# linyicheng1/trackingBench-SLAM

Hardware: AMD Instinct MI355X
Metric: frames/sec end-to-end (extract+match+local-BA) (higher is better)
Workload: dtype u8 (pyramid/FAST/ORB/Hamming) + f64 (pose-opt/BA); 1 GPU; 1280x720 stereo, 8-level pyramid x0.8, 2000 kpts/image (FAST 80/30), searchByBF L<->R, pose-opt, 10-KF/5000-pt local BA x10 iters; distinct_synthetic_pairs=64, distinct_ba_windows=32, ba_partitions=3, ba_schedule=joined at the end of every step, parallelism=frames sharded x1, RCCL gather of tracks

## Files before the change

### trackingbench_slam_amd/csrc/k_ba.hip

```cpp
#include <mutex>
#include <type_traits>
#include "tb_internal.h"
#include "tb_device.h"
#include "tb_se3.h"
#include "tb_math.h"

#define BA_T 256
#ifndef BA_KFCH
#define BA_KFCH 512
#endif
#ifndef BA_KFBLK
#define BA_KFBLK 4
#endif
#define BA_BIG_MAXF 64
#define BA_SMALL_MAXF 10
#define BA_SORT_LDS 8192
#ifndef BA_EMAX
#define BA_EMAX 64
#endif
#ifndef BA_UPD_BATCH
#define BA_UPD_BATCH 4
#endif
#ifndef BA_PCAP
#define BA_PCAP 21
#endif

struct BaState {
    double lambda, ni, currentChi, chi0, scale_p, rho;
    int iter, qmax, status, need_lin, cur, ok2, done_iters, err;
    int sing, pad0, hq_fresh, pad2;
};

struct BaDims {
    int W, nkf, nfixed, nfree, np, npt, obs_pitch, iters;
    int nblkP, kfChunks, G, nChunks;
    int Gbase, Gextra;
    int Vbase, Vextra;
    int big, npairs;
    unsigned long long oBigA;
    unsigned long long oPairStart, oPairCnt, oPairItems, maxItems;
    double fx, fy, cx, cy;
    unsigned long long wstride, oT, oP, oHll, oBl, oHq, oHpp, oBp, oXp, oPartKF, oPartP, oPartS;
    unsigned long long istride, oPtStart, oPtFree, oKfStart, oKfEdges, oFreeKP;
    unsigned long long oKfRec;
    unsigned long long oPtMask, oPermA, oPermB, oPtRank, oKPs, oGDesc;
    unsigned long long oGCost;
    unsigned long long oGCut;
    int renum;
    unsigned long long oPerm;
    int stream;
    int schurWaveLds;
    int wgReduce;
};

__host__ __device__ inline int ba_schur_waves(const BaDims& d, int w) {
    return d.wgReduce ? 4 * (d.Gbase + (w < d.Gextra ? 1 : 0)) : d.Vbase + (w < d.Vextra ? 1 : 0);
}
__device__ __forceinline__ void ba_schur_unit(int u, int base, int extra, int& w, int& i) {
    const int head = extra * (base + 1);
    if (u < head) { w = u / (base + 1); i = u - w * (base + 1); }
    else { const int r = u - head; w = extra + r / base; i = r - (w - extra) * base; }
}

typedef double ba_d4 __attribute__((ext_vector_type(4)));
typedef double ba_d2 __attribute__((ext_vector_type(2)));

__device__ __forceinline__ double ba_huber_rho0(double c, double delta) {
    const double dsqr = delta * delta;
    return (c <= dsqr) ? c : 2 * sqrt(c) * delta - dsqr;
}
struct BaLin { double ww, e0, e1, c2, invz; double pc[3]; double Jl[6]; };
__device__ __forceinline__ double ba_rcp(double x) {
    double r = __builtin_amdgcn_rcp(x);
    r = fma(fma(-x, r, 1.0), r, r);
    r = fma(fma(-x, r, 1.0), r, r);
    return r;
}
__device__ __forceinline__ void ba_residual(const double* Rt, const double* X, float u, float v, float inv_sigma2, double fx,
                                            double fy, double cx, double cy, double delta, BaLin& L) {
#pragma unroll
    for (int i = 0; i < 3; i++) L.pc[i] = fma(Rt[3 * i + 2], X[2], fma(Rt[3 * i + 1], X[1], fma(Rt[3 * i], X[0], Rt[9 + i])));
    L.invz = ba_rcp(L.pc[2]);
    L.e0 = (double)u - fma(L.pc[0] * L.invz, fx, cx);
    L.e1 = (double)v - fma(L.pc[1] * L.invz, fy, cy);
    const double wgt = (double)inv_sigma2;
    L.c2 = fma(L.e0, wgt * L.e0, L.e1 * (wgt * L.e1));
    const double r1 = (L.c2 <= delta * delta) ? 1.0 : delta / sqrt(L.c2);
    L.ww = r1 * wgt;
}
__device__ __forceinline__ void ba_linearize(const double* Rt, const double* X, float u, float v, float inv_sigma2, double fx,
                                             double fy, double cx, double cy, double delta, BaLin& L) {
    ba_residual(Rt, X, u, v, inv_sigma2, fx, fy, cx, cy, delta, L);
    const double ax = -(L.pc[0] * L.invz) * fx, ay = -(L.pc[1] * L.invz) * fy, m = -L.invz;
#pragma unroll
    for (int c = 0; c < 3; c++) {
        L.Jl[c] = m * fma(ax, Rt[6 + c], fx * Rt[c]);
        L.Jl[3 + c] = m * fma(ay, Rt[6 + c], fy * Rt[3 + c]);
    }
}
__device__ __forceinline__ void ba_pose_to_Rt(const double* T7, double* Rt) {
    PoSE3 s;
    s.qx = T7[0]; s.qy = T7[1]; s.qz = T7[2]; s.qw = T7[3]; s.tx = T7[4]; s.ty = T7[5]; s.tz = T7[6];
    po_to_R(s, Rt);
    Rt[9] = s.tx; Rt[10] = s.ty; Rt[11] = s.tz;
}
__device__ __forceinline__ void ba_jac_pose_iz(const double* pc, double invz, double fx, double fy, double* J) {
    const double xz = pc[0] * invz, yz = pc[1] * invz, xf = xz * fx, yf = yz * fy;
    J[0] = xf * yz; J[1] = -fma(xf, xz, fx); J[2] = yz * fx;
    J[3] = -invz * fx; J[4] = 0; J[5] = xf * invz;
    J[6] = fma(yf, yz, fy); J[7] = -(xz * yf); J[8] = -xz * fy;
    J[9] = 0; J[10] = -invz * fy; J[11] = yf * invz;
}

__device__ __forceinline__ bool ba_inv3(const double* H6, double lambda, double* I) {
    const double A0 = H6[0] + lambda, A1 = H6[1], A2 = H6[2], A4 = H6[3] + lambda, A5 = H6[4], A8 = H6[5] + lambda;
    const double A3 = A1, A6 = A2, A7 = A5;
    const double det = A0 * (A4 * A8 - A5 * A7) - A1 * (A3 * A8 - A5 * A6) + A2 * (A3 * A7 - A4 * A6);
    if (!(fabs(det) > 0)) return false;
    const double id = 1.0 / det;
    I[0] = (A4 * A8 - A5 * A7) * id; I[1] = (A2 * A7 - A1 * A8) * id; I[2] = (A1 * A5 - A2 * A4) * id;
    I[3] = (A5 * A6 - A3 * A8) * id; I[4] = (A0 * A8 - A2 * A6) * id; I[5] = (A2 * A3 - A0 * A5) * id;
    I[6] = (A3 * A7 - A4 * A6) * id; I[7] = (A1 * A6 - A0 * A7) * id; I[8] = (A0 * A4 - A1 * A3) * id;
    return true;
}
__device__ __forceinline__ PoSE3 ba_load_se3(const double* p) {
    PoSE3 s;
    s.qx = p[0]; s.qy = p[1]; s.qz = p[2]; s.qw = p[3]; s.tx = p[4]; s.ty = p[5]; s.tz = p[6];
    return s;
}
__device__ __forceinline__ void ba_store_se3(double* p, const PoSE3& s) {
    p[0] = s.qx; p[1] = s.qy; p[2] = s.qz; p[3] = s.qw; p[4] = s.tx; p[5] = s.ty; p[6] = s.tz;
}
__device__ __forceinline__ double ba_block_sum1(double v, double* red) {
    const int wave = threadIdx.x >> 6, lane = threadIdx.x & 63;
    v = po_wave_sum(v);
    __syncthreads();
    if (lane == 0) red[wave] = v;
    __syncthreads();
    return (red[0] + red[1]) + (red[2] + red[3]);
}
__device__ __forceinline__ double ba_block_max1(double v, double* red) {
    const int wave = threadIdx.x >> 6, lane = threadIdx.x & 63;
#pragma unroll
    for (int d = 32; d > 0; d >>= 1) v = fmax(v, __shfl_xor(v, d, 64));
    __syncthreads();
    if (lane == 0) red[wave] = v;
    __syncthreads();
    return fmax(fmax(red[0], red[1]), fmax(red[2], red[3]));
}

template <class Pred, class Pred2, class Visit>
__device__ __forceinline__ int ba_ordered_rank(int n, int* tmp, Pred pred, Pred2 pred2, int* total2, Visit visit) {
    const int wave = threadIdx.x >> 6, lane = threadIdx.x & 63;
    const int q = (((n + 3) >> 2) + 63) & ~63, lo = min(wave * q, n), hi = min(lo + q, n);
    int cnt = 0, cnt2 = 0;
    for (int e0 = lo; e0 < hi; e0 += 256) {
#pragma unroll
        for (int i = 0; i < 4; i++) {
            const int e = e0 + 64 * i + lane;
            cnt += (e < hi && pred(e)) ? 1 : 0;
            cnt2 += (e < hi && pred2(e)) ? 1 : 0;
        }
    }
    cnt = tb_wave_sum(cnt);
    cnt2 = tb_wave_sum(cnt2);
    if (lane == 0) { tmp[wave] = cnt; tmp[4 + wave] = cnt2; }
    __syncthreads();
    int base = 0;
    for (int v = 0; v < wave; v++) base += tmp[v];
    const int total = tmp[0] + tmp[1] + tmp[2] + tmp[3];
    *total2 = tmp[4] + tmp[5] + tmp[6] + tmp[7];
    const unsigned long long lt = (lane == 0) ? 0ull : (~0ull >> (64 - lane));
    for (int e0 = lo; e0 < hi; e0 += 256) {
        bool f[4];
#pragma unroll
        for (int i = 0; i < 4; i++) { const int e = e0 + 64 * i + lane; f[i] = e < hi && pred(e); }
#pragma unroll
        for (int i = 0; i < 4; i++) {
            const int e = e0 + 64 * i + lane;
            const unsigned long long m = __ballot(f[i]);
            if (e < hi) visit(e, base + __popcll(m & lt), f[i]);
            base += __popcll(m);
        }
    }
    __syncthreads();
    return total;
}

__global__ void __launch_bounds__(BA_T)
k_ba_setup(BaDims d, const float* __restrict__ poses, const float* __restrict__ pts, const tb_ba_obs* __restrict__ obsOrig,
           const tb_ba_obs* __restrict__ obsAll, const int32_t* __restrict__ obsCounts, double* __restrict__ dw, int* __restrict__ iw,
           BaState* __restrict__ states, int* __restrict__ errflag) {
    __shared__ int tmp[8];
    const int w = blockIdx.y, k = blockIdx.x, tid = threadIdx.x;
    const tb_ba_obs* obs = obsOrig + (size_t)w * d.obs_pitch;
    const int nobs = min(obsCounts[w], d.obs_pitch);
    double* D = dw + (size_t)w * d.wstride;
    int* I = iw + (size_t)w * d.istride;
    BaState* st = states + w;
    {
        const int nb = gridDim.x, per = (nobs + nb - 1) / nb;
        bool bad = false;
        for (int e = k * per + tid; e < min((k + 1) * per, nobs); e += BA_T) {
            const tb_ba_obs o = obs[e];
            if (o.kf < 0 || o.kf >= d.nkf || o.pt < 0 || o.pt >= d.npt || (e > 0 && o.pt < obs[e - 1].pt)) bad = true;
            for (int b0 = 1; b0 <= d.nkf && b0 <= e; b0 += 8) {
                int pk[8], pp[8];
#pragma unroll
                for (int i = 0; i < 8; i++) { const int ee = max(e - b0 - i, 0); pk[i] = obs[ee].kf; pp[i] = obs[ee].pt; }
#pragma unroll
                for (int i = 0; i < 8; i++)
                    if (b0 + i <= d.nkf && b0 + i <= e && pp[i] == o.pt && pk[i] == o.kf) bad = true;
                if (pp[7] != o.pt) break;
            }
        }
        if (bad) errflag[w] = 1;
    }
    obs = obsAll + (size_t)w * d.obs_pitch;
    if (d.renum && k != d.nkf) return;
    if (k < d.nkf) {
        int base = 0;
        const int mine = ba_ordered_rank(nobs, tmp, [&](int e) { return obs[e].kf == k; },
                                         [&](int e) { const int kf = obs[e].kf; return kf >= 0 && kf < k; }, &base,
                                         [&](int e, int rank, bool hit) {
                                             if (hit) {
                                                 I[d.oKfEdges + base + rank] = e;
                                                 const tb_ba_obs o = obs[e];
                                                 int4 r;
                                                 r.x = o.pt; r.y = __float_as_int(o.u); r.z = __float_as_int(o.v); r.w = __float_as_int(o.inv_sigma2);
                                                 *reinterpret_cast<int4*>(I + d.oKfRec + 4 * (size_t)(base + rank)) = r;
                                             }
                                         });
        if (tid == 0) {
            I[d.oKfStart + k] = base;
            if (k == d.nkf - 1) I[d.oKfStart + d.nkf] = base + mine;
        }
        return;
    }
    if (k == d.nkf + 1) {
        int unused = 0;
        const int nfreeE = ba_ordered_rank(nobs, tmp, [&](int e) { return obs[e].kf >= d.nfixed; }, [](int) { return false; }, &unused,
            [&](int e, int ce, bool hit) {
                const int prev = (e > 0) ? obs[e - 1].pt : -1, cur = obs[e].pt;
                for (int p = max(prev + 1, 0); p <= min(cur, d.npt); p++) I[d.oPtFree + p] = ce;
                if (hit) {
                    const tb_ba_obs o = obs[e];
                    int4 r;
                    r.x = (int)(((unsigned)cur << 6) | ((unsigned)(o.kf - d.nfixed) & 63u));
                    r.y = __float_as_int(o.u); r.z = __float_as_int(o.v); r.w = __float_as_int(o.inv_sigma2);
                    *reinterpret_cast<int4*>(I + d.oFreeKP + 4 * (size_t)ce) = r;
                }
            });
        for (int p = max((nobs > 0 ? obs[nobs - 1].pt : -1) + 1, 0) + tid; p <= d.npt; p += BA_T) I[d.oPtFree + p] = nfreeE;
        return;
    }
    if (tid == 0) {
        st->lambda = 0; st->ni = 2; st->currentChi = 0; st->chi0 = 0; st->scale_p = 0; st->rho = 0;
// ... 23 lines not shown
        D[d.oP + i] = v;
        D[d.oP + (size_t)d.npt * 3 + i] = v;
    }
}

__device__ __forceinline__ void ba_write_rec(double* q, const double* Hll, const double* bl, const double* X, double lambda,
                                             BaState* st) {
    const double a00 = Hll[0] + lambda, a10 = Hll[1], a20 = Hll[2], a11 = Hll[3] + lambda, a21 = Hll[4], a22 = Hll[5] + lambda;
    bool ok = a00 > 0;
    const double i00 = 1.0 / sqrt(ok ? a00 : 1.0), c10 = a10 * i00, c20 = a20 * i00;
    const double d1 = a11 - c10 * c10;
    ok = ok && d1 > 0;
    const double i11 = 1.0 / sqrt(ok ? d1 : 1.0), c21 = (a21 - c20 * c10) * i11;
    const double d2 = a22 - c20 * c20 - c21 * c21;
    ok = ok && d2 > 0 && isfinite(d2);
    const double i22 = 1.0 / sqrt(ok ? d2 : 1.0);
    if (!ok) st->sing = 1;
    const double u00 = i00, u11 = i11, u22 = i22, u01 = -c10 * i00 * i11, u12 = -c21 * i11 * i22,
                 u02 = -(c20 * i00 + c21 * u01) * i22;
    ba_d2* q2 = reinterpret_cast<ba_d2*>(q);
    q2[0] = ba_d2{ok ? u00 : 0.0, ok ? u01 : 0.0};
    q2[1] = ba_d2{ok ? u02 : 0.0, ok ? u11 : 0.0};
    q2[2] = ba_d2{ok ? u12 : 0.0, ok ? u22 : 0.0};
    q2[3] = ba_d2{bl[0], bl[1]};
    q2[4] = ba_d2{bl[2], X[0]};
    q2[5] = ba_d2{X[1], X[2]};
}
__device__ __forceinline__ void ba_load_rec(const double* __restrict__ q, double* __restrict__ r) {
    const ba_d2* q2 = reinterpret_cast<const ba_d2*>(q);
#pragma unroll
    for (int i = 0; i < 6; i++) { const ba_d2 v = q2[i]; r[2 * i] = v.x; r[2 * i + 1] = v.y; }
}

struct BaStreamPos { int base, deg; int4 first; };
template <class F>
__device__ __forceinline__ void ba_stream_walk(const int4* __restrict__ S, const BaStreamPos& sp, F f) {
    const int deg = sp.deg;
    int base = sp.base;
    unsigned long long m = __ballot(0 < deg);
    int4 rn = sp.first;
    for (int j = 0; m != 0; j++) {
        const int4 r = rn;
        const unsigned long long mn = __ballot(j + 1 < deg);
        const int idx = tbm::ba_stream_slot_self(mn, &base);
        if (j + 1 < deg) rn = S[idx];
        if (j < deg) f(r);
        m = mn;
    }
}
template <int N, class F>
__device__ __forceinline__ void ba_stream_walk_batched(const int4* __restrict__ S, const BaStreamPos& sp, F f) {
    const int deg = sp.deg;
    int base = sp.base - __popcll(__ballot(0 < deg));
    for (int j0 = 0; __ballot(j0 < deg) != 0; j0 += N) {
        int4 r[N];
#pragma unroll
        for (int i = 0; i < N; i++) {
            const unsigned long long m = __ballot(j0 + i < deg);
            const int idx = tbm::ba_stream_slot_self(m, &base);
            r[i] = make_int4(0, 0, 0, 0);
            if (j0 + i < deg) r[i] = S[idx];
        }
#pragma unroll
        for (int i = 0; i < N; i++)
            if (j0 + i < deg) f(r[i]);
    }
}
__device__ __forceinline__ BaStreamPos ba_stream_begin(const BaDims& d, const int* __restrict__ I, int p) {
    BaStreamPos sp;
    sp.base = I[d.oPtStart + min(p & ~63, d.npt)];
    sp.deg = (p < d.npt) ? I[d.oPtStart + p + 1] - I[d.oPtStart + p] : 0;
    sp.first = make_int4(0, 0, 0, 0);
    const int idx = tbm::ba_stream_slot_self(__ballot(0 < sp.deg), &sp.base);
    if (0 < sp.deg) sp.first = reinterpret_cast<const int4*>(I + d.oFreeKP)[idx];
    return sp;
}

__device__ __forceinline__ void ba_rec_utb(const double* q, double* t) {
    t[0] = q[0] * q[6];
    t[1] = q[1] * q[6] + q[3] * q[7];
    t[2] = q[2] * q[6] + q[4] * q[7] + q[5] * q[8];
}

template <bool STREAM>
__device__ __forceinline__ void ba_points_pass(const BaDims& d, const tb_ba_obs* __restrict__ obsAll, double* __restrict__ dw, const int* __restrict__ iw,
                                               BaState* __restrict__ states, const int* __restrict__ errflag, int bx, int w) {
    __shared__ double red[4];
    extern __shared__ __attribute__((aligned(16))) double sRt[];
    const int tid = threadIdx.x;
    double* D = dw + (size_t)w * d.wstride;
    const int* I = iw + (size_t)w * d.istride;
    const int p = bx * BA_T + tid;
    BaStreamPos sp;
    if (STREAM) sp = ba_stream_begin(d, I, p);
    if (errflag[w]) {
        if (bx == 0 && tid == 0) { states[w].status = 1; states[w].err = 1; }
        return;
    }
    const BaState st = states[w];
    if (st.status) return;
    const bool lam_known = st.iter > 0 || !st.need_lin;
    const tb_ba_obs* obs = obsAll + (size_t)w * d.obs_pitch;
    const double* T = D + d.oT + (size_t)st.cur * d.nkf * 7;
    const double* P = D + d.oP + (size_t)st.cur * d.npt * 3;
    for (int k = tid; k < d.nkf; k += BA_T) ba_pose_to_Rt(T + k * 7, sRt + k * 12);
    __syncthreads();
    const double delta = (double)sqrtf(5.991f);
    const bool in = p < d.npt;
    double chi = 0, maxd = 0;
    double Hll[6] = {0, 0, 0, 0, 0, 0}, bl[3] = {0, 0, 0}, X[3] = {0, 0, 0};
    if (in) { X[0] = P[3 * p]; X[1] = P[3 * p + 1]; X[2] = P[3 * p + 2]; }
    auto edge = [&](int kf, float ou, float ov, float ow) {
        BaLin L;
        ba_linearize(sRt + kf * 12, X, ou, ov, ow, d.fx, d.fy, d.cx, d.cy, delta, L);
        const double ww = L.ww, e0 = L.e0, e1 = L.e1;
        const double* Jl = L.Jl;
        chi += ba_huber_rho0(L.c2, delta);
        for (int a = 0; a < 3; a++) bl[a] = fma(-ww, fma(Jl[a], e0, Jl[3 + a] * e1), bl[a]);
        Hll[0] = fma(ww, fma(Jl[0], Jl[0], Jl[3] * Jl[3]), Hll[0]);
        Hll[1] = fma(ww, fma(Jl[0], Jl[1], Jl[3] * Jl[4]), Hll[1]);
        Hll[2] = fma(ww, fma(Jl[0], Jl[2], Jl[3] * Jl[5]), Hll[2]);
        Hll[3] = fma(ww, fma(Jl[1], Jl[1], Jl[4] * Jl[4]), Hll[3]);
        Hll[4] = fma(ww, fma(Jl[1], Jl[2], Jl[4] * Jl[5]), Hll[4]);
        Hll[5] = fma(ww, fma(Jl[2], Jl[2], Jl[5] * Jl[5]), Hll[5]);
    };
    if (STREAM) {
        ba_stream_walk(reinterpret_cast<const int4*>(I + d.oFreeKP), sp,
                       [&](const int4& r) { edge(r.x, __int_as_float(r.y), __int_as_float(r.z), __int_as_float(r.w)); });
    } else if (in) {
        const int eBeg = I[d.oPtStart + p], eEnd = I[d.oPtStart + p + 1];
        tb_ba_obs on = obs[min(eBeg, d.obs_pitch - 1)];
        for (int e = eBeg; e < eEnd; e++) {
            const tb_ba_obs o = on;
            on = obs[min(e + 1, d.obs_pitch - 1)];
            edge(o.kf, o.u, o.v, o.inv_sigma2);
        }
    }
    if (in) {
        if (!lam_known) {
            for (int a = 0; a < 6; a++) D[d.oHll + (size_t)p * 6 + a] = Hll[a];
            for (int a = 0; a < 3; a++) D[d.oBl + (size_t)p * 3 + a] = bl[a];
        } else
            ba_write_rec(D + d.oHq + (size_t)(d.renum ? p : I[d.oPtRank + p]) * 12, Hll, bl, X, st.lambda, states + w);
        maxd = fmax(fabs(Hll[0]), fmax(fabs(Hll[3]), fabs(Hll[5])));
    }
    const double s = ba_block_sum1(chi, red);
    const double m = ba_block_max1(maxd, red);
    if (tid == 0) {
        D[d.oPartP + (size_t)bx * 4] = s;
        D[d.oPartP + (size_t)bx * 4 + 1] = m;
    }
}

#define BA_KFG 14
#define BA_KFR_LDS (4 * (BA_KFG * 65 + 64) + 4 * 27)
__device__ __forceinline__ double ba_block_sum27(const double (&v)[27], double* sh) {
    const int tid = threadIdx.x, wave = tid >> 6, lane = tid & 63;
    double* T = sh + wave * (BA_KFG * 65 + 64);
    double* Qs = T + BA_KFG * 65;
    double* red = sh + 4 * (BA_KFG * 65 + 64);
#pragma unroll
    for (int g = 0; g < (27 + BA_KFG - 1) / BA_KFG; g++) {
        const int nv = min(BA_KFG, 27 - BA_KFG * g);
#pragma unroll
        for (int i = 0; i < BA_KFG; i++)
            if (i < nv) T[i * 65 + lane] = v[BA_KFG * g + i];
        __builtin_amdgcn_fence(__ATOMIC_SEQ_CST, "wavefront");
        const int q = lane / BA_KFG, i = lane - BA_KFG * q;
        if (lane < 4 * BA_KFG && i < nv) {
            const double* src = T + i * 65 + 16 * q;
            double s = src[0];
#pragma unroll
            for (int k = 1; k < 16; k++) s += src[k];
            Qs[lane] = s;
        }
        __builtin_amdgcn_fence(__ATOMIC_SEQ_CST, "wavefront");
        if (lane < nv) red[wave * 27 + BA_KFG * g + lane] = (Qs[lane] + Qs[BA_KFG + lane]) + (Qs[2 * BA_KFG + lane] + Qs[3 * BA_KFG + lane]);
        __builtin_amdgcn_fence(__ATOMIC_SEQ_CST, "wavefront");
    }
    __syncthreads();
    double r = 0;
    if (tid < 27) r = (red[tid] + red[27 + tid]) + (red[54 + tid] + red[81 + tid]);
    __syncthreads();
    return r;
}

__device__ __forceinline__ void ba_kf_pass(const BaDims& d, const tb_ba_obs* __restrict__ obsAll, double* __restrict__ dw, const int* __restrict__ iw,
                                           const BaState* __restrict__ states, const int* __restrict__ errflag, int bid) {
    __shared__ double red[BA_KFR_LDS];
    const int tid = threadIdx.x, nx = min(BA_KFBLK, d.kfChunks), per = nx * d.nfree;
    const int run = bid / (8 * per), rr_ = bid - run * (8 * per);
    const int w = run * 8 + (rr_ & 7), slot = rr_ >> 3;
    if (w >= d.W) return;
    if (errflag[w]) return;
    const int chunk0 = slot % nx, kfree = slot / nx, kf = d.nfixed + kfree;
    const BaState st = states[w];
    if (st.status || !st.need_lin) return;
    double* D = dw + (size_t)w * d.wstride;
    const int* I = iw + (size_t)w * d.istride;
    const int beg = I[d.oKfStart + kf], end = I[d.oKfStart + kf + 1];
    double Tk[12];
    ba_pose_to_Rt(D + d.oT + ((size_t)st.cur * d.nkf + kf) * 7, Tk);
    const double* P = D + d.oP + (size_t)st.cur * d.npt * 3;
    const double delta = (double)sqrtf(5.991f);
    for (int chunk = chunk0; chunk * BA_KFCH < end - beg; chunk += BA_KFBLK) {
        double acc[27];
#pragma unroll
        for (int i = 0; i < 27; i++) acc[i] = 0;
        int4 rr[BA_KFCH / BA_T];
        double XX[BA_KFCH / BA_T][3];
        const int4* KR = reinterpret_cast<const int4*>(I + d.oKfRec);
#pragma unroll
        for (int j = 0; j < BA_KFCH / BA_T; j++) {
            const int idx = beg + chunk * BA_KFCH + j * BA_T + tid;
            rr[j] = KR[min(idx, end - 1)];
            if (idx >= end) rr[j].x = -1;
        }
#pragma unroll
        for (int j = 0; j < BA_KFCH / BA_T; j++) {
            const int p = min(max(rr[j].x, 0), d.npt - 1);
            XX[j][0] = P[3 * p]; XX[j][1] = P[3 * p + 1]; XX[j][2] = P[3 * p + 2];
        }
#pragma unroll
        for (int j = 0; j < BA_KFCH / BA_T; j++) {
            if (rr[j].x < 0) continue;
            const float ou = __int_as_float(rr[j].y), ov = __int_as_float(rr[j].z), ow = __int_as_float(rr[j].w);
            const double* X = XX[j];
            double Jp[12];
            BaLin L;
            ba_residual(Tk, X, ou, ov, ow, d.fx, d.fy, d.cx, d.cy, delta, L);
            ba_jac_pose_iz(L.pc, L.invz, d.fx, d.fy, Jp);
            const double ww = L.ww, e0 = L.e0, e1 = L.e1;
#pragma unroll
            for (int a = 0; a < 6; a++) {
                const double wa = ww * Jp[a], wb = ww * Jp[6 + a];
                acc[21 + a] -= fma(wa, e0, wb * e1);
#pragma unroll
                for (int c = a; c < 6; c++) {
                    const int at = a * 6 - (a * (a - 1)) / 2 + (c - a);
                    acc[at] += fma(wa, Jp[c], wb * Jp[6 + c]);
                }
            }
        }
        const double tot = ba_block_sum27(acc, red);
        if (tid < 27) D[d.oPartKF + ((size_t)kfree * d.kfChunks + chunk) * 27 + tid] = tot;
    }
}

template <bool STREAM>
__global__ void __launch_bounds__(BA_T)
k_ba_points(BaDims d, const tb_ba_obs* __restrict__ obsAll, double* __restrict__ dw, const int* __restrict__ iw, BaState* __restrict__ states,
            const int* __restrict__ errflag) {
    ba_points_pass<STREAM>(d, obsAll, dw, iw, states, errflag, (int)blockIdx.x, (int)blockIdx.y);
}
__global__ void __launch_bounds__(BA_T)
k_ba_kf(BaDims d, const tb_ba_obs* __restrict__ obsAll, double* __restrict__ dw, const int* __restrict__ iw, const BaState* __restrict__ states,
        const int* __restrict__ errflag) {
    ba_kf_pass(d, obsAll, dw, iw, states, errflag, (int)blockIdx.x);
}
template <bool STREAM>
__global__ void __launch_bounds__(BA_T)
k_ba_lin(BaDims d, const tb_ba_obs* __restrict__ obsAll, double* __restrict__ dw, const int* __restrict__ iw, BaState* __restrict__ states,
         const int* __restrict__ errflag, int nKfBlocks) {
    if ((int)blockIdx.x < nKfBlocks) ba_kf_pass(d, obsAll, dw, iw, states, errflag, (int)blockIdx.x);
    else {
        const int b = (int)blockIdx.x - nKfBlocks;
        ba_points_pass<STREAM>(d, obsAll, dw, iw, states, errflag, b % d.nblkP, b / d.nblkP);
    }
}

__device__ __forceinline__ void ba_reduce_body(const BaDims& d, double* __restrict__ dw, const int* __restrict__ iw, BaState* __restrict__ states,
                                               int w, double* red) {
    const int tid = threadIdx.x;
    BaState* st = states + w;
    double* D = dw + (size_t)w * d.wstride;
    const int* I = iw + (size_t)w * d.istride;
    double maxd = 0;
    for (int i = tid; i < d.nfree * 27; i += BA_T) {
        const int kf = i / 27, c = i - kf * 27;
        const int nedges = I[d.oKfStart + d.nfixed + kf + 1] - I[d.oKfStart + d.nfixed + kf];
        const int nch = (nedges + BA_KFCH - 1) / BA_KFCH;
        double s = 0;
        for (int ch = 0; ch < nch; ch++) s += D[d.oPartKF + ((size_t)kf * d.kfChunks + ch) * 27 + c];
        if (c >= 21) D[d.oBp + kf * 6 + (c - 21)] = s;
        else {
            int a = 0, rem = c;
            while (rem >= 6 - a) { rem -= 6 - a; a++; }
            const int b = a + rem;
            D[d.oHpp + (size_t)kf * 36 + a * 6 + b] = s;
            D[d.oHpp + (size_t)kf * 36 + b * 6 + a] = s;
            if (a == b) maxd = fmax(maxd, fabs(s));
        }
    }
    const double mH = ba_block_max1(maxd, red);
    if (tid == 0) {
        double chi = 0, mL = 0;
        for (int b = 0; b < d.nblkP; b++) { chi += D[d.oPartP + (size_t)b * 4]; mL = fmax(mL, D[d.oPartP + (size_t)b * 4 + 1]); }
        st->currentChi = chi;
        if (st->iter == 0) { st->chi0 = chi; st->lambda = 1e-5 * fmax(mH, mL); st->ni = 2; }
        st->hq_fresh = st->iter > 0 ? 1 : 0;
        st->need_lin = 0;
    }
}

__global__ void __launch_bounds__(BA_T)
k_ba_reduce(BaDims d, double* __restrict__ dw, const int* __restrict__ iw, BaState* __restrict__ states) {
    __shared__ double red[4];
    const int w = blockIdx.x;
    if (states[w].status || !states[w].need_lin) return;
    ba_reduce_body(d, dw, iw, states, w, red);
}

__global__ void __launch_bounds__(BA_T)
k_ba_hinv(BaDims d, double* __restrict__ dw, const int* __restrict__ iw, BaState* __restrict__ states) {
    const int w = blockIdx.y, p = blockIdx.x * BA_T + threadIdx.x;
    const BaState st = states[w];
    if (st.status || st.hq_fresh || p >= d.npt) return;
    double* D = dw + (size_t)w * d.wstride;
    const int* I = iw + (size_t)w * d.istride;
    double ph[6], pb[3], X[3];
#pragma unroll
    for (int i = 0; i < 6; i++) ph[i] = D[d.oHll + (size_t)p * 6 + i];
#pragma unroll
    for (int i = 0; i < 3; i++) { pb[i] = D[d.oBl + (size_t)p * 3 + i]; X[i] = D[d.oP + ((size_t)st.cur * d.npt + p) * 3 + i]; }
    ba_write_rec(D + d.oHq + (size_t)(d.renum ? p : I[d.oPtRank + p]) * 12, ph, pb, X, st.lambda, states + w);
}

#define BA_MAXT 4
#define BA_REC 12
#define BA_RECS_LDS 256
#define BA_KMFMA 5
#define BA_ZERO_LDS 40
__device__ __forceinline__ void ba_wave_lds_fence() { __builtin_amdgcn_fence(__ATOMIC_SEQ_CST, "wavefront"); }

__host__ __device__ constexpr int ba_c_cap(int k) { return (BA_EMAX / k) < BA_PCAP ? (BA_EMAX / k) : BA_PCAP; }
__host__ __device__ constexpr int ba_c_nb(int k) { return (6 * k + 1 + 3) / 4; }
__host__ __device__ constexpr int ba_c_ld(int k) { return ((3 * ba_c_cap(k) + 3) / 4) * 4 + 2; }
__host__ __device__ constexpr int ba_c_tile(int k) { return 4 * ba_c_nb(k) * ba_c_ld(k); }
#define BA_CB 37
__host__ __device__ constexpr int ba_c_rhs(int k) { return BA_CB * (k * (k + 1) / 2); }
__host__ __device__ constexpr int ba_c_tri(int k) { return ba_c_rhs(k) + 6 * k; }
__host__ __device__ constexpr int ba_c_nacc(int k) {
    const int nb = ba_c_nb(k), nvf = nb / 4, rem = nb % 4;
    return 3 * nvf + 2 * nvf * (nvf - 1) + rem * (nvf + 1);
}
struct BaCTab { int cap[BA_SMALL_MAXF + 1], ld[BA_SMALL_MAXF + 1], nacc[BA_SMALL_MAXF + 1]; };
__host__ __device__ constexpr BaCTab ba_c_tab() {
    BaCTab t = {};
    for (int k = 1; k <= BA_SMALL_MAXF; k++) { t.cap[k] = ba_c_cap(k); t.ld[k] = ba_c_ld(k); t.nacc[k] = ba_c_nacc(k); }
    return t;
}
__device__ const BaCTab ba_ctab = ba_c_tab();
static int ba_c_wave_lds(int nfree) {
    int m = 0;
    for (int k = 1; k <= nfree; k++) m = std::max(m, std::max(ba_c_tile(k), k <= BA_KMFMA ? ba_c_tri(k) : 0));
    return ((m + 3) & ~3) + BA_RECS_LDS + BA_ZERO_LDS;
}

template <class IsZero>
__device__ __forceinline__ void ba_stable_split(int n, int* tmp, const int* src, int* dst, IsZero isZero) {
    const int wave = threadIdx.x >> 6, lane = threadIdx.x & 63;
    const int q = (((n + 3) >> 2) + 63) & ~63, lo = min(wave * q, n), hi = min(lo + q, n);
    int cnt = 0;
    for (int e = lo + lane; e < hi; e += 64) cnt += isZero(src[e]) ? 1 : 0;
    cnt = tb_wave_sum(cnt);
    if (lane == 0) tmp[wave] = cnt;
    __syncthreads();
    int z = 0;
    for (int v = 0; v < wave; v++) z += tmp[v];
    int o = (tmp[0] + tmp[1] + tmp[2] + tmp[3]) + (lo - z);
    const unsigned long long lt = (lane == 0) ? 0ull : (~0ull >> (64 - lane));
    for (int e0 = lo; e0 < hi; e0 += 64) {
        const int e = e0 + lane;
        const bool valid = e < hi;
        const int v = valid ? src[e] : 0;
        const bool f = valid && isZero(v);
        const unsigned long long m0 = __ballot(f), m1 = __ballot(valid && !f);
        if (valid) dst[f ? z + __popcll(m0 & lt) : o + __popcll(m1 & lt)] = v;
        z += __popcll(m0);
        o += __popcll(m1);
    }
    __threadfence_block();
    __syncthreads();
}

#define BA_RT 1024
#define BA_PREP_MAXKF 64
__global__ void __launch_bounds__(BA_RT)
k_ba_prepare(BaDims d, const tb_ba_obs* __restrict__ obsAll, const int32_t* __restrict__ obsCounts, int* __restrict__ iw,
             tb_ba_obs* __restrict__ obs2All) {
    extern __shared__ __attribute__((aligned(16))) unsigned prep_lds[];
    unsigned* word = prep_lds;
    int* first = reinterpret_cast<int*>(prep_lds + d.npt);
    int* start2 = first + d.npt;
    unsigned short* pbuf = reinterpret_cast<unsigned short*>(start2 + d.npt + 1);
    constexpr int NW = BA_RT / 64;
    __shared__ int tmp[NW + 2];
    __shared__ int bins[1 << BA_SMALL_MAXF];
    __shared__ int kfc[NW][BA_PREP_MAXKF];
    const int w = blockIdx.x, tid = threadIdx.x, wave = tid >> 6, lane = tid & 63;
    const unsigned long long lt = (lane == 0) ? 0ull : (~0ull >> (64 - lane));
    const tb_ba_obs* obs = obsAll + (size_t)w * d.obs_pitch;
    tb_ba_obs* obs2 = obs2All + (size_t)w * d.obs_pitch;
    const int nobs = min(max(obsCounts[w], 0), d.obs_pitch);
    int* I = iw + (size_t)w * d.istride;
    for (int p = tid; p < d.npt; p += BA_RT) { word[p] = 0; first[p] = 0; }
    for (int i = tid; i < (1 << BA_SMALL_MAXF); i += BA_RT) bins[i] = 0;
    __syncthreads();
    for (int e0 = tid; e0 < nobs; e0 += 4 * BA_RT) {
        tb_ba_obs o[4];
        int prev[4];
#pragma unroll
        for (int i = 0; i < 4; i++) {
            const int e = min(e0 + i * BA_RT, nobs - 1);
// ... 1486 lines not shown
static void ba_dims(BaDims& d, int num_cu, int peers, int W, const double K[4], int nkf, int nfixed, int npt, int obs_pitch, int iters) {
    memset(&d, 0, sizeof d);
    d.W = W; d.nkf = nkf; d.nfixed = nfixed; d.nfree = nkf - nfixed; d.np = 6 * d.nfree; d.npt = npt; d.obs_pitch = obs_pitch;
    d.iters = iters;
    d.nblkP = (npt + BA_T - 1) / BA_T;
    d.kfChunks = (obs_pitch + BA_KFCH - 1) / BA_KFCH;
    d.nChunks = 0;
    {
        const int slots = std::max(2 * std::max(num_cu, 1) / std::max(peers, 1), 1), cap = std::min(32, std::max((npt / 64 + 3) / 4, 1));
        d.Gbase = std::min(std::max(slots / std::max(W, 1), 1), cap);
        d.Gextra = (d.Gbase < cap && slots > d.Gbase * W) ? std::min(slots - d.Gbase * W, W) : 0;
        d.G = d.Gbase + (d.Gextra > 0 ? 1 : 0);
        d.wgReduce = d.Gbase > 4 ? 1 : 0;
        const int T = 4 * std::max(slots, W);
        d.Vbase = std::min(T / std::max(W, 1), 4 * cap);
        d.Vextra = d.Vbase < 4 * cap ? T % std::max(W, 1) : 0;
    }
    d.big = d.nfree > BA_SMALL_MAXF;
    d.renum = (!d.big && npt <= BA_SORT_LDS && nkf <= BA_PREP_MAXKF) ? 1 : 0;
    d.stream = d.renum;
    d.schurWaveLds = d.big ? 0 : ba_c_wave_lds(d.nfree);
    d.npairs = d.nfree * (d.nfree + 1) / 2;
    d.maxItems = (unsigned long long)obs_pitch * (d.nfree + 1) / 2 + 1;
    d.fx = K[0]; d.fy = K[1]; d.cx = K[2]; d.cy = K[3];
    unsigned long long o = 0;
    auto take = [&](unsigned long long n) { unsigned long long r = o; o += (n + 1) & ~1ull; return r; };
    d.oT = take(2ull * nkf * 7);
    d.oP = take(2ull * npt * 3);
    d.oHll = take(6ull * npt);
    d.oBl = take(3ull * npt);
    d.oHq = take(12ull * npt);
    d.oHpp = take(36ull * std::max(d.nfree, 1));
    d.oBp = take(std::max(64, d.np));
    d.oXp = take(std::max(64, d.np));
    d.oPartKF = take(27ull * std::max(d.nfree, 1) * d.kfChunks);
    d.oPartP = take(4ull * d.nblkP);
    const int maxWaves = d.wgReduce ? 4 * d.G : d.Vbase + (d.Vextra > 0 ? 1 : 0);
    d.oPartS = take(d.big ? 0 : 4096ull * (d.wgReduce ? d.G : maxWaves));
    d.oBigA = take(d.big ? (unsigned long long)(d.np + 1) * d.np + 32 : 0);
    d.wstride = o;
    unsigned long long io = 0;
    auto itake = [&](unsigned long long n) { unsigned long long r = io; io += (n + 3) & ~3ull; return r; };
    d.oPtStart = itake(npt + 1);
    d.oPtFree = itake(npt + 1);
    d.oKfStart = itake(nkf + 1);
    d.oKfEdges = itake(obs_pitch);
    d.oFreeKP = itake(4ull * obs_pitch);
    d.oKfRec = itake(4ull * obs_pitch);
    d.oPtRank = itake(npt);
    d.oPerm = itake(d.renum ? npt : 0);
    d.oPtMask = itake(d.big ? 0 : npt);
    d.oPermA = itake(d.big ? 0 : npt);
    d.oPermB = itake(d.big ? 0 : npt);
    d.oKPs = itake(d.big ? 0 : 4ull * obs_pitch);
    d.oGDesc = itake(d.big ? 0 : 4ull * npt + 4);
    d.oGCost = itake(d.big ? 0 : (unsigned long long)npt + 1);
    d.oGCut = itake(d.big ? 0 : (unsigned long long)maxWaves + 1);
    d.oPairStart = itake(d.big ? d.npairs + 1 : 0);
    d.oPairCnt = itake(d.big ? d.npairs : 0);
    d.oPairItems = itake(d.big ? 2 * d.maxItems : 0);
    d.istride = io;
}

#define BA_RING 1000

struct BaPlan {
    BaDims d;
    float *poses, *pts;
    const tb_ba_obs* obs_in;
    const int32_t* counts;
    void* work;
    double* dw;
    int* iw;
    BaState* states;
    int *running, *errflag;
    tb_ba_obs* obs2;
    size_t work_bytes;
    const tb_ba_obs* obs;
    decltype(&k_ba_schur_c<1>) schur;
    decltype(&k_ba_solve<16>) solve;
    decltype(&k_ba_lin<true>) lin;
    decltype(&k_ba_points<true>) points;
    decltype(&k_ba_update<true>) update;
    size_t prepare_lds, pass_lds, schur_lds, big_lds, update_lds;
};

static BaPlan ba_plan(const tb_ctx* ctx, int W, const double K[4], int nkf, int nfixed, int npt, int obs_pitch, int iters, float* d_poses,
                      float* d_pts, const tb_ba_obs* d_obs, const int32_t* d_counts, void* d_work) {
    BaPlan p;
    BaDims& d = p.d;
    ba_dims(d, ctx->num_cu, ctx->peers, W, K, nkf, nfixed, npt, obs_pitch, iters);
    if (ctx->dbg_ba_plain_obs) d.stream = 0;
    p.poses = d_poses; p.pts = d_pts; p.obs_in = d_obs; p.counts = d_counts; p.work = d_work;
    uintptr_t at = (uintptr_t)d_work;
    size_t total = 0;
    auto take = [&](size_t bytes, size_t align) {
        at = (at + align - 1) / align * align;
        const uintptr_t r = at;
        at += bytes;
        total += bytes + (align > 1 ? align : 0);
        return r;
    };
    p.dw = (double*)take((size_t)W * d.wstride * sizeof(double), 1);
    p.iw = (int*)take((size_t)W * d.istride * sizeof(int), 1);
    p.states = (BaState*)take((size_t)W * sizeof(BaState), 1);
    p.running = (int*)take(BA_RING * sizeof(int), 1);
    p.errflag = (int*)take((size_t)W * sizeof(int), 1);
    p.obs2 = d.renum ? (tb_ba_obs*)take((size_t)W * obs_pitch * sizeof(tb_ba_obs), 64) : nullptr;
    p.work_bytes = total + 96;
    p.obs = d.renum ? p.obs2 : d_obs;
    const int R = (d.np + 15) >> 4;
    p.schur = R == 1 ? k_ba_schur_c<1> : R == 2 ? k_ba_schur_c<2> : R == 3 ? k_ba_schur_c<3> : k_ba_schur_c<4>;
    p.solve = d.np <= 16 ? k_ba_solve<16> : d.np <= 32 ? k_ba_solve<32> : d.np <= 48 ? k_ba_solve<48> : k_ba_solve<64>;
    p.lin = d.stream ? k_ba_lin<true> : k_ba_lin<false>;
    p.points = d.stream ? k_ba_points<true> : k_ba_points<false>;
    p.update = d.stream ? k_ba_update<true> : k_ba_update<false>;
    p.prepare_lds = (size_t)npt * 16 + 16;
    p.pass_lds = (size_t)d.nkf * 12 * sizeof(double);
    p.schur_lds = std::max<size_t>(4 * (size_t)d.schurWaveLds, d.wgReduce ? 64 * 64 : 0) * sizeof(double);
    p.big_lds = (size_t)(d.np + 1) * BA_PLD * sizeof(double);
    p.update_lds = ((size_t)d.nkf * 24 + d.np) * sizeof(double);
    return p;
}

size_t tbk_local_ba_work_bytes(const tb_ctx* ctx, int W, int nkf, int nfixed, int npt, int obs_pitch) {
    const double K[4] = {1, 1, 0, 0};
    return ba_plan(ctx, W, K, nkf, nfixed, npt, obs_pitch, 1, nullptr, nullptr, nullptr, nullptr, nullptr).work_bytes;
}

static int ba_enqueue_head(tb_ctx* ctx, const BaPlan& p) {
    const BaDims& d = p.d;
    const int W = d.W;
    TB_TRY(tb_launch(ctx, nullptr, k_ba_zero, dim3((BA_RING + W + 255) / 256), dim3(256), 0, p.running, BA_RING + W));
    if (d.renum) TB_TRY(tb_launch(ctx, "k_ba_prepare", k_ba_prepare, dim3(W), dim3(BA_RT), p.prepare_lds, d, p.obs_in, p.counts, p.iw, p.obs2));
    TB_TRY(tb_launch(ctx, "k_ba_setup", k_ba_setup, dim3(d.nkf + 2, W), dim3(BA_T), 0, d, p.poses, p.pts, p.obs_in, p.obs, p.counts, p.dw, p.iw,
                     p.states, p.errflag));
    if (d.renum) {
    } else if (!d.big) {
        TB_TRY(tb_launch(ctx, "k_ba_groups", k_ba_groups, dim3(W), dim3(BA_T), 0, d, p.iw, p.errflag));
    } else {
        tb_prof_begin(ctx, "k_ba_pairs");
        TB_TRY(tb_launch(ctx, nullptr, k_ba_pairs<false>, dim3(d.nfree, W), dim3(64), 0, d, p.obs, p.iw, p.errflag));
        TB_TRY(tb_launch(ctx, nullptr, k_ba_pair_scan, dim3(W), dim3(BA_T), 0, d, p.iw, p.errflag));
        TB_TRY(tb_launch(ctx, nullptr, k_ba_pairs<true>, dim3(d.nfree, W), dim3(64), 0, d, p.obs, p.iw, p.errflag));
        tb_prof_end(ctx);
    }
    return TB_OK;
}

static int ba_enqueue_round(tb_ctx* ctx, const BaPlan& p, int round) {
    const BaDims& d = p.d;
    const int W = d.W;
    const int nKfBlocks = ((W + 7) / 8) * 8 * std::min(BA_KFBLK, d.kfChunks) * d.nfree;
    if (W <= 32) {
        TB_TRY(tb_launch(ctx, "k_ba_lin", p.lin, dim3(nKfBlocks + d.nblkP * W), dim3(BA_T), p.pass_lds, d, p.obs, p.dw, p.iw, p.states, p.errflag,
                         nKfBlocks));
    } else {
        TB_TRY(tb_launch(ctx, "k_ba_points", p.points, dim3(d.nblkP, W), dim3(BA_T), p.pass_lds, d, p.obs, p.dw, p.iw, p.states, p.errflag));
        TB_TRY(tb_launch(ctx, "k_ba_kf", k_ba_kf, dim3(nKfBlocks), dim3(BA_T), 0, d, p.obs, p.dw, p.iw, p.states, p.errflag));
    }
    const bool reduce_in_solve = !d.big && round > 0;
    if (!reduce_in_solve) TB_TRY(tb_launch(ctx, "k_ba_reduce", k_ba_reduce, dim3(W), dim3(BA_T), 0, d, p.dw, p.iw, p.states));
    if (round == 0)
        TB_TRY(tb_launch(ctx, "k_ba_hinv", k_ba_hinv, dim3(d.nblkP, W), dim3(BA_T), 0, d, p.dw, p.iw, p.states));
    if (d.big) {
        TB_TRY(tb_launch(ctx, "k_ba_schur_pairs", k_ba_schur_pairs, dim3((d.npairs + 3) / 4, W), dim3(BA_T), 0, d, p.dw, p.iw, p.states));
        TB_TRY(tb_launch(ctx, "k_ba_solve_big", k_ba_solve_big, dim3(W), dim3(BA_ST), p.big_lds, d, p.dw, p.states));
    } else {
        TB_TRY(tb_launch(ctx, "k_ba_schur", p.schur, dim3(d.wgReduce ? d.Gbase * W + d.Gextra : (d.Vbase * W + d.Vextra + 3) / 4), dim3(BA_T),
                         p.schur_lds, d, p.dw, p.iw, p.states));
        TB_TRY(tb_launch(ctx, "k_ba_solve", p.solve, dim3(W), dim3(BA_SOLVE_T), 0, d, p.dw, p.iw, p.states, reduce_in_solve ? 1 : 0));
    }
    TB_TRY(tb_launch(ctx, "k_ba_update", p.update, dim3(d.nblkP, W), dim3(BA_T), p.update_lds, d, p.obs, p.dw, p.iw, p.states));
    return tb_launch(ctx, "k_ba_decide", k_ba_decide, dim3(W), dim3(64), 0, d, p.dw, p.states, p.running + round % BA_RING);
}

static int ba_graph(tb_ctx* ctx, const BaPlan& p, int nfirst, hipGraphExec_t* exec) {
    struct Key { BaDims d; const void *poses, *pts, *obs, *counts, *work; hipStream_t s; } key;
    memset(&key, 0, sizeof key);
    key.d = p.d; key.poses = p.poses; key.pts = p.pts; key.obs = p.obs_in; key.counts = p.counts; key.work = p.work; key.s = ctx->stream;
    const std::string kb((const char*)&key, sizeof key);
    for (auto& g : ctx->ba_graphs)
        if (g.first == kb) { *exec = g.second; return TB_OK; }
    static std::mutex capture_lock;
    std::lock_guard<std::mutex> guard(capture_lock);
    hipGraph_t graph = nullptr;
    TB_HIP(ctx, hipStreamBeginCapture(ctx->stream, hipStreamCaptureModeThreadLocal));
    int rc = ba_enqueue_head(ctx, p);
    for (int r = 0; r < nfirst && rc == TB_OK; r++) rc = ba_enqueue_round(ctx, p, r);
    const hipError_t e = hipStreamEndCapture(ctx->stream, &graph);
    if (rc != TB_OK) { if (graph) hipGraphDestroy(graph); return rc; }
    TB_HIP(ctx, e);
    const hipError_t e2 = hipGraphInstantiate(exec, graph, nullptr, nullptr, 0);
    hipGraphDestroy(graph);
    TB_HIP(ctx, e2);
    if (ctx->ba_graphs.size() >= 8) {
        hipGraphExecDestroy(ctx->ba_graphs.front().second);
        ctx->ba_graphs.erase(ctx->ba_graphs.begin());
    }
    ctx->ba_graphs.emplace_back(kb, *exec);
    return TB_OK;
}

int tbk_local_ba_batch(tb_ctx* ctx, int W, const double K[4], int nkf, int nfixed, float* d_poses, int npt, float* d_pts,
                       const tb_ba_obs* d_obs, const int32_t* d_counts, int obs_pitch, int iters, double* d_stats, void* d_work,
                       size_t work_bytes) {
    if (W <= 0) return TB_OK;
    const int nfree = nkf - nfixed;
    if (nfree < 1 || nfree > BA_BIG_MAXF)
        return tb_fail(ctx, TB_EUNSUPPORTED, "local BA: %d free keyframes (this build supports 1..64)", nfree);
    if (nkf > TB_MAX_LEVELS * 8) return tb_fail(ctx, TB_EUNSUPPORTED, "local BA: too many keyframes");
    if (npt > (1 << 25)) return tb_fail(ctx, TB_EUNSUPPORTED, "local BA: more than 2^25 points per window");
    if (nfree > BA_SMALL_MAXF && (unsigned long long)obs_pitch * (nfree + 1) >= (1ull << 31))
        return tb_fail(ctx, TB_EUNSUPPORTED, "local BA: large window with more than 2^31 / (free keyframes + 1) observations");
    if (iters > 99) return tb_fail(ctx, TB_EUNSUPPORTED, "local BA: more than 99 LM iterations (one still-running counter per trial, 1000 of them)");
    const BaPlan p = ba_plan(ctx, W, K, nkf, nfixed, npt, obs_pitch, iters, d_poses, d_pts, d_obs, d_counts, d_work);
    const BaDims& d = p.d;
    if (p.work_bytes > work_bytes) return tb_fail(ctx, TB_ENOMEM, "local BA workspace too small");
    hipStream_t s = ctx->stream;
    if (!d.big) TB_TRY(tb_lds_limit(ctx, (const void*)p.schur, p.schur_lds));
    if (d.renum) TB_TRY(tb_lds_limit(ctx, (const void*)k_ba_prepare, p.prepare_lds));
    if (d.big) TB_TRY(tb_lds_limit(ctx, (const void*)k_ba_solve_big, p.big_lds));
    const int max_rounds = std::min(iters * 10 + 1, BA_RING);
    int batch = iters;
    const int nfirst = std::min(batch, max_rounds);
    const bool use_graph = W <= 32 && !ctx->prof && nfirst > 0;
    int rounds = 0;
    if (use_graph) {
        hipGraphExec_t exec = nullptr;
        TB_TRY(ba_graph(ctx, p, nfirst, &exec));
        TB_HIP(ctx, hipGraphLaunch(exec, s));
        rounds = nfirst;
    } else {
        TB_TRY(ba_enqueue_head(ctx, p));
    }
    int host_running = nfirst > 0 ? 1 : 0;
    bool replayed = use_graph;
    while (host_running > 0 && (rounds < max_rounds || replayed)) {
        if (!replayed)
            for (int r = 0; r < batch && rounds < max_rounds; r++, rounds++) TB_TRY(ba_enqueue_round(ctx, p, rounds));
        replayed = false;
        TB_HIP(ctx, hipMemcpyAsync(&host_running, p.running + (rounds - 1) % BA_RING, sizeof(int), hipMemcpyDeviceToHost, s));
        TB_HIP(ctx, hipStreamSynchronize(s));
        batch = 4;
    }
    return tb_launch(ctx, "k_ba_finish", k_ba_finish, dim3(W), dim3(BA_T), 0, d, p.dw, p.iw, p.states, d_poses, d_pts, d_stats);
}
```

Measured before the change: 34190 frames/s.

## Restructure BA keyframe pass into contiguous chunk ranges with prefetch pipelining

The keyframe Hessian pass now gives each block a contiguous range of chunks (one block per keyframe by default) instead of striding chunks across four blocks. Within that range it streams edge records through a two-deep software prefetch of records and point gathers, accumulating into a single register accumulator. The keyframe pose is computed once per block, shared through LDS and made wave-uniform with readfirstlane. The reduction group size is shrunk, launch bounds now request occupancy, and unused partial slots are zeroed. This is meant to cut redundant reductions and latency stalls, at the cost of fewer blocks and less parallelism per keyframe.

```diff
diff --git a/trackingbench_slam_amd/csrc/k_ba.hip b/trackingbench_slam_amd/csrc/k_ba.hip
--- a/trackingbench_slam_amd/csrc/k_ba.hip
+++ b/trackingbench_slam_amd/csrc/k_ba.hip
@@ -10,7 +10,19 @@
 #define BA_KFCH 512
 #endif
 #ifndef BA_KFBLK
-#define BA_KFBLK 4
+#define BA_KFBLK 1
+#endif
+#ifndef BA_KFE
+#define BA_KFE 2
+#endif
+#ifndef BA_LIN_FUSE_ALL
+#define BA_LIN_FUSE_ALL 0
+#endif
+#ifndef BA_KF_AHEAD
+#define BA_KF_AHEAD 1
+#endif
+#ifndef BA_KF_POSE_ONCE
+#define BA_KF_POSE_ONCE 1
 #endif
 #define BA_BIG_MAXF 64
 #define BA_SMALL_MAXF 10
@@ -103,6 +115,10 @@
     s.qx = T7[0]; s.qy = T7[1]; s.qz = T7[2]; s.qw = T7[3]; s.tx = T7[4]; s.ty = T7[5]; s.tz = T7[6];
     po_to_R(s, Rt);
     Rt[9] = s.tx; Rt[10] = s.ty; Rt[11] = s.tz;
+}
+__device__ __forceinline__ double ba_uniform(double v) {
+    const int lo = __builtin_amdgcn_readfirstlane(__double2loint(v)), hi = __builtin_amdgcn_readfirstlane(__double2hiint(v));
+    return __hiloint2double(hi, lo);
 }
 __device__ __forceinline__ void ba_jac_pose_iz(const double* pc, double invz, double fx, double fy, double* J) {
     const double xz = pc[0] * invz, yz = pc[1] * invz, xf = xz * fx, yf = yz * fy;
@@ -432,13 +448,16 @@
     }
 }
 
-#define BA_KFG 14
-#define BA_KFR_LDS (4 * (BA_KFG * 65 + 64) + 4 * 27)
+#ifndef BA_KFG
+#define BA_KFG 4
+#endif
+#define BA_KFW_LDS (BA_KFG * 65 + 4 * BA_KFG)
+#define BA_KFR_LDS (4 * BA_KFW_LDS + 4 * 27)
 __device__ __forceinline__ double ba_block_sum27(const double (&v)[27], double* sh) {
     const int tid = threadIdx.x, wave = tid >> 6, lane = tid & 63;
-    double* T = sh + wave * (BA_KFG * 65 + 64);
+    double* T = sh + wave * BA_KFW_LDS;
     double* Qs = T + BA_KFG * 65;
-    double* red = sh + 4 * (BA_KFG * 65 + 64);
+    double* red = sh + 4 * BA_KFW_LDS;
 #pragma unroll
     for (int g = 0; g < (27 + BA_KFG - 1) / BA_KFG; g++) {
         const int nv = min(BA_KFG, 27 - BA_KFG * g);
@@ -467,44 +486,67 @@
 
 __device__ __forceinline__ void ba_kf_pass(const BaDims& d, const tb_ba_obs* __restrict__ obsAll, double* __restrict__ dw, const int* __restrict__ iw,
                                            const BaState* __restrict__ states, const int* __restrict__ errflag, int bid) {
-    __shared__ double red[BA_KFR_LDS];
+    __shared__ double red[BA_KFR_LDS + 12];
     const int tid = threadIdx.x, nx = min(BA_KFBLK, d.kfChunks), per = nx * d.nfree;
     const int run = bid / (8 * per), rr_ = bid - run * (8 * per);
     const int w = run * 8 + (rr_ & 7), slot = rr_ >> 3;
     if (w >= d.W) return;
     if (errflag[w]) return;
-    const int chunk0 = slot % nx, kfree = slot / nx, kf = d.nfixed + kfree;
+    const int share = slot % nx, kfree = slot / nx, kf = d.nfixed + kfree;
     const BaState st = states[w];
     if (st.status || !st.need_lin) return;
     double* D = dw + (size_t)w * d.wstride;
     const int* I = iw + (size_t)w * d.istride;
     const int beg = I[d.oKfStart + kf], end = I[d.oKfStart + kf + 1];
+    const int nch = (end - beg + BA_KFCH - 1) / BA_KFCH, cps = (nch + nx - 1) / nx;
+    const int c0 = share * cps, c1 = min(c0 + cps, nch);
+    if (c0 >= c1) return;
+    const int eb = beg + c0 * BA_KFCH, ee = min(beg + c1 * BA_KFCH, end);
     double Tk[12];
+#if BA_KF_POSE_ONCE
+    double* sRt = red + BA_KFR_LDS;
+    if (tid < 64) {
+        ba_pose_to_Rt(D + d.oT + ((size_t)st.cur * d.nkf + kf) * 7, Tk);
+        if (tid == 0) {
+#pragma unroll
+            for (int i = 0; i < 12; i++) sRt[i] = Tk[i];
+        }
+    }
+    __syncthreads();
+#pragma unroll
+    for (int i = 0; i < 12; i++) Tk[i] = ba_uniform(sRt[i]);
+#else
     ba_pose_to_Rt(D + d.oT + ((size_t)st.cur * d.nkf + kf) * 7, Tk);
+#pragma unroll
+    for (int i = 0; i < 12; i++) Tk[i] = ba_uniform(Tk[i]);
+#endif
     const double* P = D + d.oP + (size_t)st.cur * d.npt * 3;
     const double delta = (double)sqrtf(5.991f);
-    for (int chunk = chunk0; chunk * BA_KFCH < end - beg; chunk += BA_KFBLK) {
-        double acc[27];
-#pragma unroll
-        for (int i = 0; i < 27; i++) acc[i] = 0;
-        int4 rr[BA_KFCH / BA_T];
-        double XX[BA_KFCH / BA_T][3];
-        const int4* KR = reinterpret_cast<const int4*>(I + d.oKfRec);
-#pragma unroll
-        for (int j = 0; j < BA_KFCH / BA_T; j++) {
-            const int idx = beg + chunk * BA_KFCH + j * BA_T + tid;
-            rr[j] = KR[min(idx, end - 1)];
-            if (idx >= end) rr[j].x = -1;
-        }
-#pragma unroll
-        for (int j = 0; j < BA_KFCH / BA_T; j++) {
-            const int p = min(max(rr[j].x, 0), d.npt - 1);
-            XX[j][0] = P[3 * p]; XX[j][1] = P[3 * p + 1]; XX[j][2] = P[3 * p + 2];
-        }
-#pragma unroll
-        for (int j = 0; j < BA_KFCH / BA_T; j++) {
-            if (rr[j].x < 0) continue;
-            const float ou = __int_as_float(rr[j].y), ov = __int_as_float(rr[j].z), ow = __int_as_float(rr[j].w);
+    const int4* KR = reinterpret_cast<const int4*>(I + d.oKfRec);
+    const int nr = (ee - eb + BA_KFE * BA_T - 1) / (BA_KFE * BA_T);
+    auto load_rec = [&](int r, int4 (&rec)[BA_KFE]) {
+#pragma unroll
+        for (int j = 0; j < BA_KFE; j++) {
+            const int idx = eb + (r * BA_KFE + j) * BA_T + tid;
+            rec[j] = KR[min(idx, ee - 1)];
+            if (idx >= ee) rec[j].x = -1;
+        }
+    };
+    auto gather = [&](const int4 (&rec)[BA_KFE], double (&X)[BA_KFE][3]) {
+#pragma unroll
+        for (int j = 0; j < BA_KFE; j++) {
+            const int p = min(max(rec[j].x, 0), d.npt - 1);
+            X[j][0] = P[3 * p]; X[j][1] = P[3 * p + 1]; X[j][2] = P[3 * p + 2];
+        }
+    };
+    double acc[27];
+#pragma unroll
+    for (int i = 0; i < 27; i++) acc[i] = 0;
+    auto edges = [&](const int4 (&rec)[BA_KFE], const double (&XX)[BA_KFE][3]) {
+#pragma unroll
+        for (int j = 0; j < BA_KFE; j++) {
+            if (rec[j].x < 0) continue;
+            const float ou = __int_as_float(rec[j].y), ov = __int_as_float(rec[j].z), ow = __int_as_float(rec[j].w);
             const double* X = XX[j];
             double Jp[12];
             BaLin L;
@@ -522,8 +564,39 @@
                 }
             }
         }
-        const double tot = ba_block_sum27(acc, red);
-        if (tid < 27) D[d.oPartKF + ((size_t)kfree * d.kfChunks + chunk) * 27 + tid] = tot;
+    };
+#if BA_KF_AHEAD
+    int4 ra[BA_KFE], rb[BA_KFE];
+    double Xa[BA_KFE][3];
+    load_rec(0, ra);
+    load_rec(1, rb);
+    gather(ra, Xa);
+    for (int r = 0; r < nr; r++) {
+        int4 rc[BA_KFE];
+        double Xb[BA_KFE][3];
+        gather(rb, Xb);
+        load_rec(r + 2, rc);
+        edges(ra, Xa);
+#pragma unroll
+        for (int j = 0; j < BA_KFE; j++) {
+            ra[j] = rb[j]; rb[j] = rc[j];
+            Xa[j][0] = Xb[j][0]; Xa[j][1] = Xb[j][1]; Xa[j][2] = Xb[j][2];
+        }
+    }
+#else
+    for (int r = 0; r < nr; r++) {
+        int4 ra[BA_KFE];
+        double Xa[BA_KFE][3];
+        load_rec(r, ra);
+        gather(ra, Xa);
+        edges(ra, Xa);
+    }
+#endif
+    const double tot = ba_block_sum27(acc, red);
+    if (tid < 27) {
+        double* out = D + d.oPartKF + ((size_t)kfree * d.kfChunks + c0) * 27 + tid;
+        out[0] = tot;
+        for (int ch = 1; ch < c1 - c0; ch++) out[ch * 27] = 0.0;
     }
 }
 
@@ -533,13 +606,13 @@
             const int* __restrict__ errflag) {
     ba_points_pass<STREAM>(d, obsAll, dw, iw, states, errflag, (int)blockIdx.x, (int)blockIdx.y);
 }
-__global__ void __launch_bounds__(BA_T)
+__global__ void __launch_bounds__(BA_T, 4)
 k_ba_kf(BaDims d, const tb_ba_obs* __restrict__ obsAll, double* __restrict__ dw, const int* __restrict__ iw, const BaState* __restrict__ states,
         const int* __restrict__ errflag) {
     ba_kf_pass(d, obsAll, dw, iw, states, errflag, (int)blockIdx.x);
 }
 template <bool STREAM>
-__global__ void __launch_bounds__(BA_T)
+__global__ void __launch_bounds__(BA_T, 4)
 k_ba_lin(BaDims d, const tb_ba_obs* __restrict__ obsAll, double* __restrict__ dw, const int* __restrict__ iw, BaState* __restrict__ states,
          const int* __restrict__ errflag, int nKfBlocks) {
     if ((int)blockIdx.x < nKfBlocks) ba_kf_pass(d, obsAll, dw, iw, states, errflag, (int)blockIdx.x);
@@ -2332,7 +2405,7 @@
     const BaDims& d = p.d;
     const int W = d.W;
     const int nKfBlocks = ((W + 7) / 8) * 8 * std::min(BA_KFBLK, d.kfChunks) * d.nfree;
-    if (W <= 32) {
+    if (W <= 32 || BA_LIN_FUSE_ALL) {
         TB_TRY(tb_launch(ctx, "k_ba_lin", p.lin, dim3(nKfBlocks + d.nblkP * W), dim3(BA_T), p.pass_lds, d, p.obs, p.dw, p.iw, p.states, p.errflag,
                          nKfBlocks));
     } else {
```

Measured after the change: 36040 frames/s, median of 6. 5.4% higher.
